# jayin92/Skyfall-GS

Hardware: AMD Instinct MI355X
Metric: train-step Gaussians/s (fwd+bwd raster) @1080p (higher is better)
Workload: dtype f32; 1 GPU; configs[1]: synthetic cfg2 scene (SURVEY 8d), N=2000000 Gaussians/GPU, 1920x1080, z ~ U(250, 350), colors_precomp, kernel_size=0.1, subpixel_offset=zeros[H,W,2], dL/dimage and dL/ddepth ~ N(0,1)/P, seed=rank, one scene per GPU; N=2000000, width=1920, height=1080, N_vis=2000000, D_ref_16x16=5856939, D_binned_8x8=6945415, parallelism=scene-per-gpu x1, prewarm_steps=50, settle_steps=0, order=random

## Files before the change

### skyfall-gs_amd/csrc/raster_bwd.hip

```cpp
#include <cstring>

#include "act_math.h"
#include "sfgs_internal.h"

namespace sfgs {

__global__ void __launch_bounds__(256)
dupgrad_prefill_kernel(int T8, const uint16_t* __restrict__ tile_dead, unsigned long long n_dup, int mode,
                       uint4* __restrict__ live16, uint4* __restrict__ zero_line, unsigned long long* __restrict__ hdr,
                       unsigned long long* __restrict__ feedback, const unsigned long long* __restrict__ dup_pool,
                       unsigned long long dup_capacity, unsigned npools) {
  __shared__ unsigned part[4];
  unsigned dead = 0;
  unsigned long long dead64 = 0ull;
  const uint4* v = reinterpret_cast<const uint4*>(tile_dead);
  const int n8 = T8 / 8;
  for (int i = threadIdx.x; i < n8; i += 256) {
    const uint4 q = v[i];
    dead += (q.x & 0xffffu) + (q.x >> 16) + (q.y & 0xffffu) + (q.y >> 16) + (q.z & 0xffffu) + (q.z >> 16) +
            (q.w & 0xffffu) + (q.w >> 16);
    if (dead > 0x7fffffffu) { dead64 += dead; dead = 0; }
  }
  for (int t = n8 * 8 + threadIdx.x; t < T8; t += 256) dead += tile_dead[t];
  dead64 += dead;
// ... 61 lines not shown
    __syncthreads();
    if (lane == 0) {
#pragma unroll
      for (int i = 0; i < NF; ++i) part[wave][i] = v[i];
    }
    __syncthreads();
    if (threadIdx.x < NF) {
      const float s = ((part[0][threadIdx.x] + part[1][threadIdx.x]) + part[2][threadIdx.x]) + part[3][threadIdx.x];
      reinterpret_cast<float*>(dupgrad + d0 * DG_F4)[threadIdx.x] = s;
    }
  }
}

struct DupAcc {
  float4 q[DG_F4];
  __device__ __forceinline__ void zero() {
#pragma unroll
    for (int i = 0; i < DG_F4; ++i) q[i] = make_float4(0.f, 0.f, 0.f, 0.f);
  }
  __device__ __forceinline__ void add(const float4* __restrict__ r) {
#pragma unroll
    for (int i = 0; i < DG_F4; ++i) {
      const float4 x = r[i];
      q[i].x += x.x; q[i].y += x.y; q[i].z += x.z;
      if (DG_F4 == 3) q[i].w += x.w;
    }
  }
  __device__ __forceinline__ float get(int f) const {
    if constexpr (DG_F4 == 3) { const float4 v = q[f >> 2]; const int c = f & 3; return c == 0 ? v.x : c == 1 ? v.y : c == 2 ? v.z : v.w; }
    else { const float4 v = q[f & 3]; const int c = f >> 2; return c == 0 ? v.x : c == 1 ? v.y : v.z; }
  }
};

template <int K, int DEG, bool RAW, int CMX>
__global__ void __launch_bounds__(PRE_BLOCK)
preprocess_bwd_kernel(KFrame kf, int N, const float* __restrict__ means3D, const float* __restrict__ scales,
                      const float* __restrict__ rots, const void* __restrict__ opac_, const void* __restrict__ filt,
                      int raw_mask, const float* __restrict__ shs, const float* __restrict__ shs_rest,
                      const float* __restrict__ sh_dirs, int dirs_are_centers,
                      const int* __restrict__ radii,
                      const uint2* __restrict__ dup, const float4* __restrict__ dupgrad, const uint8_t* __restrict__ live,
                      size_t zero_f4, const unsigned long long* __restrict__ hdr,
                      float* __restrict__ g_means3D, float* __restrict__ g_means2D, float* __restrict__ g_scales,
                      float* __restrict__ g_rots, void* __restrict__ g_opac_, float* __restrict__ g_colors,
                      float* __restrict__ g_shs, float* __restrict__ g_shs_rest, float* __restrict__ g_sh_dirs) {
  constexpr bool SPLIT = CMX >= 3;
  constexpr int CM = SPLIT ? CMX - 3 : CMX;
  static_assert(!SPLIT || (K > 1 && CM != 1), "split SH storage: more than one coefficient, coefficient-major");
  constexpr int PB_CHUNK = 128;
  static_assert((PB_CHUNK * DG_F4) % 64 == 0, "whole load rounds");
  __shared__ float4 pb_stage[PRE_BLOCK / 64][PB_CHUNK * DG_F4];
  const int g = blockIdx.x * PRE_BLOCK + threadIdx.x;
  const bool valid = g < N;
  const int lane = threadIdx.x & 63;
  constexpr unsigned COOP = 32;
  const bool vis = valid && radii[g] > 0;
  unsigned d0 = 0, cnt = 0;
  if (vis) { const uint2 dr = dup[g]; d0 = dr.x; cnt = dr.y; }
  const bool flags = live != nullptr && hdr[HDR_PREFILLED] != 0ull;
  DupAcc acc;
  acc.zero();
  if (cnt > BWD_BIG) {
    for (unsigned d = d0; d < d0 + cnt; d += BWD_CHUNK) acc.add(dupgrad + (size_t)d * DG_F4);
  }
  {
    const bool small = cnt > 0 && cnt <= COOP;
    const unsigned rb = small ? d0 : 0xffffffffu, re = small ? d0 + cnt : 0u;
    unsigned w0 = rb, w1 = re;
#pragma unroll
    for (int d = 32; d >= 1; d >>= 1) {
      w0 = min(w0, (unsigned)__shfl_xor((int)w0, d));
      w1 = max(w1, (unsigned)__shfl_xor((int)w1, d));
    }
    float4* stage = pb_stage[threadIdx.x >> 6];
    for (unsigned c0 = w0; c0 < w1; c0 += PB_CHUNK) {
      const unsigned c1 = min(c0 + PB_CHUNK, w1);
      if (__ballot(small && rb < c1 && re > c0) == 0ull) continue;
      const unsigned n4 = (c1 - c0) * DG_F4;
      constexpr int NLD = PB_CHUNK * DG_F4 / 64;
      float4 tmp[NLD];
      size_t src[NLD];
#pragma unroll
      for (int k = 0; k < NLD; ++k) src[k] = (size_t)c0 * DG_F4 + min((unsigned)(k * 64 + lane), n4 - 1u);
      if (flags) {
        static_assert(DG_F4 == 3, "piece -> record: u / 3");
        unsigned char lv[NLD];
#pragma unroll
        for (int k = 0; k < NLD; ++k) lv[k] = live[(size_t)c0 + min((unsigned)(k * 64 + lane), n4 - 1u) / 3u];
        unsigned any = 0;
#pragma unroll
        for (int k = 0; k < NLD; ++k) { src[k] = lv[k] ? src[k] : zero_f4; any |= lv[k]; }
        if (__ballot(any != 0u) == 0ull) continue;
      }
#pragma unroll
      for (int k = 0; k < NLD; ++k) tmp[k] = dupgrad[src[k]];
#pragma unroll
      for (int k = 0; k < NLD; ++k) stage[k * 64 + lane] = tmp[k];
      __builtin_amdgcn_wave_barrier();
      __builtin_amdgcn_fence(__ATOMIC_ACQ_REL, "wavefront");
      if (small) {
        const unsigned lo = max(rb, c0), hi = min(re, c1);
        for (unsigned d = lo; d < hi; ++d) acc.add(stage + (size_t)(d - c0) * DG_F4);
      }
      __builtin_amdgcn_wave_barrier();
      __builtin_amdgcn_fence(__ATOMIC_ACQ_REL, "wavefront");
    }
  }
  for (unsigned long long todo = __ballot(cnt > COOP && cnt <= BWD_BIG); todo; todo &= todo - 1) {
    const int src = __builtin_ctzll(todo);
    const unsigned b0 = (unsigned)__shfl((int)d0, src), bn = (unsigned)__shfl((int)cnt, src);
    DupAcc w;
    w.zero();
    if (flags) {
      constexpr int U = 4;
      for (unsigned r = 0; r < bn; r += 64 * U) {
        bool lv[U];
        bool any = false;
#pragma unroll
        for (int j = 0; j < U; ++j) {
          const unsigned i = r + 64u * j + lane;
          lv[j] = live[(size_t)b0 + min(i, bn - 1u)] != 0 && i < bn;
          any |= lv[j];
        }
        if (__ballot(any) == 0ull) continue;
#pragma unroll
        for (int j = 0; j < U; ++j)
          if (lv[j]) w.add(dupgrad + (size_t)(b0 + r + 64u * j + lane) * DG_F4);
      }
    } else {
      for (unsigned i = lane; i < bn; i += 64) w.add(dupgrad + (size_t)(b0 + i) * DG_F4);
    }
#pragma unroll
    for (int i = 0; i < DG_F4; ++i) {
#pragma unroll
      for (int d = 32; d >= 1; d >>= 1) {
        w.q[i].x += __shfl_xor(w.q[i].x, d); w.q[i].y += __shfl_xor(w.q[i].y, d); w.q[i].z += __shfl_xor(w.q[i].z, d);
        if (DG_F4 == 3) w.q[i].w += __shfl_xor(w.q[i].w, d);
      }
    }
    if (lane == src) acc = w;
  }
  if (!valid) return;
  FrameParams f = load_frame(kf);
  f.sh_degree = DEG; f.sh_coeffs = K;
  GaussGrads out;
#pragma unroll
  for (int i = 0; i < 3; ++i) { out.means3D[i] = 0.f; out.means2D[i] = 0.f; out.scales[i] = 0.f; out.rgb[i] = 0.f; }
#pragma unroll
  for (int i = 0; i < 4; ++i) out.rot[i] = 0.f;
  out.opacity = 0.f;
  constexpr int ROW = K > 0 ? 3 * K : 1;
  float gshl[ROW];
#pragma unroll
  for (int i = 0; i < ROW; ++i) gshl[i] = 0.f;
  float gdir[3] = {0.f, 0.f, 0.f};
  if (vis) {
    GradSums A;
    A.x = acc.get(0); A.y = acc.get(1); A.ax = acc.get(2); A.ay = acc.get(3);
    A.xx = acc.get(4); A.xy = acc.get(5); A.yy = acc.get(6); A.u = acc.get(7);
    A.r = acc.get(8); A.g = acc.get(9); A.b = acc.get(10); A.d = acc.get(11);
    float p[3], s[3];
    load3(means3D + 3 * (size_t)g, p);
    load3(scales + 3 * (size_t)g, s);
    const float4 qraw = *reinterpret_cast<const float4*>(rots + 4 * (size_t)g);
    float4 qv = qraw;
    float opacity;
    const float sraw[3] = {s[0], s[1], s[2]};
    unsigned long long o_bits = 0ull, f_bits = 0ull;
    if constexpr (!RAW) {
      opacity = static_cast<const float*>(opac_)[g];
    } else {
#define SFGS_ACT_LOAD(FT, OT) do { o_bits = raw_bits<OT>(opac_, g); f_bits = raw_bits<FT>(filt, g); } while (0)
      SFGS_ACT_DISPATCH(raw_mask, SFGS_ACT_LOAD);
#undef SFGS_ACT_LOAD
#define SFGS_ACT_FWD(FT, OT) act_outputs(act_terms<FT, OT>(sraw, from_bits<OT>(o_bits), from_bits<FT>(f_bits)), s, &opacity)
      SFGS_ACT_DISPATCH(raw_mask, SFGS_ACT_FWD);
#undef SFGS_ACT_FWD
      qv = act_rotation(qraw);
    }
    const float q[4] = {qv.x, qv.y, qv.z, qv.w};
    if constexpr (K > 0) {
      float shl[ROW];
      if constexpr (SPLIT) load_sh_rows<K>(shs, shs_rest, (size_t)g, shl);
      else load_row<ROW>(shs + (size_t)ROW * g, shl);
      if constexpr (CM != 0) {
        float din[3];
        load3(sh_dirs + 3 * (size_t)g, din);
        preprocess_backward_sums(f, p, s, q, opacity, shl, A, out, gshl, CM == 1, dirs_are_centers ? nullptr : din, gdir,
                                 dirs_are_centers ? din : nullptr);
      } else {
        preprocess_backward_sums(f, p, s, q, opacity, shl, A, out, gshl);
      }
    } else {
      preprocess_backward_sums(f, p, s, q, opacity, nullptr, A, out, gshl);
    }
    if constexpr (RAW) {
      const float gs[3] = {out.scales[0], out.scales[1], out.scales[2]};
#define SFGS_ACT_BWD(FT, OT)                                                                                         \
  do {                                                                                                              \
    OT gro;                                                                                                         \
    act_backward(act_terms<FT, OT>(sraw, from_bits<OT>(o_bits), from_bits<FT>(f_bits)), gs, out.opacity, out.scales, \
                 &gro);                                                                                             \
    static_cast<OT*>(g_opac_)[g] = gro;                                                                             \
  } while (0)
      SFGS_ACT_DISPATCH(raw_mask, SFGS_ACT_BWD);
#undef SFGS_ACT_BWD
      const float4 gq = act_rotation_backward(qraw, make_float4(out.rot[0], out.rot[1], out.rot[2], out.rot[3]));
// ... 136 lines not shown
```

### skyfall-gs_amd/csrc/raster_preprocess.hip

```cpp
#include <algorithm>

#include "act_math.h"
#include "sfgs_internal.h"

namespace sfgs {


__global__ void __launch_bounds__(256) subpix_bound_kernel(const float* __restrict__ subpix, int64_t n,
                                                           unsigned long long* __restrict__ hdr) {
  __shared__ float s_m[4];
  float m = 0.f;
  const int64_t n4 = (reinterpret_cast<uintptr_t>(subpix) & 15) ? 0 : (n >> 2);
  const float4* __restrict__ v4 = reinterpret_cast<const float4*>(subpix);
  for (int64_t i = (int64_t)blockIdx.x * blockDim.x + threadIdx.x; i < n4; i += (int64_t)gridDim.x * blockDim.x) {
    const float4 v = v4[i];
    m = fmaxf(fmaxf(m, fmaxf(fabsf(v.x), fabsf(v.y))), fmaxf(fabsf(v.z), fabsf(v.w)));
  }
  for (int64_t i = (n4 << 2) + (int64_t)blockIdx.x * blockDim.x + threadIdx.x; i < n; i += (int64_t)gridDim.x * blockDim.x)
    m = fmaxf(m, fabsf(subpix[i]));
#pragma unroll
  for (int d = 32; d >= 1; d >>= 1) m = fmaxf(m, __shfl_xor(m, d));
  if (lane_id() == 0) s_m[threadIdx.x >> 6] = m;
  __syncthreads();
  if (threadIdx.x == 0) {
// ... 45 lines not shown
  bool hit = false;
  int cb = 0;
  if (i < ncb) {
    const int cx = a.cx0 + i % nx, cy = a.cy0 + i / nx;
    const int tx = cx * COARSE + (t & (COARSE - 1)), ty = cy * COARSE + (t / COARSE);
    cb = cy * CX + cx;
    if (tx >= a.br.x0 && tx < a.br.x1 && ty >= a.br.y0 && ty < a.br.y1) hit = bin_test(a.r, a.thr, tx, ty, W, H, bound);
  }
  *cb_index = cb;
  return __ballot(hit);
}

__device__ __forceinline__ unsigned wave_sum_u32(unsigned v) {
#pragma unroll
  for (int d = 32; d >= 1; d >>= 1) v += (unsigned)__shfl_xor((int)v, d);
  return v;
}

template <int K, int DEG, bool RAW, int CM>
__global__ void __launch_bounds__(PRE_BLOCK)
preprocess_kernel(KFrame kf, int N, const float* __restrict__ means3D, const float* __restrict__ scales,
                  const float* __restrict__ rots, const void* __restrict__ opac_, const void* __restrict__ filt,
                  int raw_mask,
                  const float* __restrict__ colors, const float* __restrict__ shs, const float* __restrict__ shs_rest,
                  const float* __restrict__ sh_dirs, int dirs_are_centers, int* __restrict__ radii,
                  float4* __restrict__ rec_out, uint2* __restrict__ dup_out, uint32_t* __restrict__ coarse_count,
                  uint4* __restrict__ slabs, unsigned coarse_capacity, unsigned long long dup_capacity,
                  uint32_t* __restrict__ block_nvis, unsigned long long* __restrict__ block_dref,
                  uint4* __restrict__ big_list, unsigned long long* __restrict__ hdr,
                  unsigned long long* __restrict__ dup_pool, uint4* __restrict__ pairs,
                  uint32_t* __restrict__ block_items) {
  __shared__ unsigned s_red[PRE_BLOCK / 64 + 1];
  __shared__ unsigned long long s_base;
  const FrameParams f = load_frame(kf);
  const float bound = __uint_as_float((unsigned)hdr[HDR_SUBPIX_BOUND]);
  const int g = blockIdx.x * PRE_BLOCK + threadIdx.x;
  const int CX = (((f.W + TILE_BIN - 1) / TILE_BIN) + COARSE - 1) / COARSE;
  unsigned n_dup = 0, vis = 0, dref = 0, depth_bits = 0;
  unsigned long long mask_lo = 0ull, mask_hi = 0ull;
  unsigned walk_tiles = 0;
  bool big = false;
  bool huge = false;
  const int lane = threadIdx.x & 63;
  SplatRec r;
  BinRange br;
  float thr = 0.f;
  int cx0 = 0, cx1 = 0, cy0 = 0, cy1 = 0;
  br.x0 = br.x1 = br.y0 = br.y1 = 0;
  if (g < N) {
    float p[3], s[3];
    load3(means3D + 3 * (size_t)g, p);
    load3(scales + 3 * (size_t)g, s);
    float4 qv = *reinterpret_cast<const float4*>(rots + 4 * (size_t)g);
    float opacity_in = 0.f;
    if constexpr (!RAW) opacity_in = static_cast<const float*>(opac_)[g];
    float rgb_in[3] = {0.f, 0.f, 0.f};
    if constexpr (K == 0) load3(colors + 3 * (size_t)g, rgb_in);
    unsigned long long o_bits = 0ull, f_bits = 0ull;
    if constexpr (RAW) {
#define SFGS_ACT_LOAD(FT, OT) do { o_bits = raw_bits<OT>(opac_, g); f_bits = raw_bits<FT>(filt, g); } while (0)
      SFGS_ACT_DISPATCH(raw_mask, SFGS_ACT_LOAD);
#undef SFGS_ACT_LOAD
    }
    asm volatile("" :: "v"(p[2]), "v"(s[0]), "v"(qv.x), "v"(opacity_in), "v"(rgb_in[0]), "v"((unsigned)o_bits),
                 "v"((unsigned)f_bits));
    if constexpr (RAW) {
// ... 111 lines not shown
      __builtin_amdgcn_wave_barrier();
    }
  }
  const unsigned long long big_lanes = __ballot(big);
  for (unsigned long long bl = big_lanes; bl; bl &= bl - 1) {
    const int L = __builtin_ctzll(bl);
    const WalkArgs a = broadcast_walk(r, br, thr, cx0, cx1, cy0, cy1, L);
    const int ncb = (a.cx1 - a.cx0) * (a.cy1 - a.cy0);
    unsigned total = 0;
    for (int it = 0; it * 4 < ncb; ++it) {
      int cb;
      total += (unsigned)__popcll(walk_ballot4(a, it, lane, f.W, f.H, bound, &cb, CX));
    }
    if (lane == L) n_dup = total;
  }
  const unsigned long long huge_lanes = __ballot(huge);
  if (huge_lanes) {
    unsigned long long slot0 = 0ull;
    if (lane == 0) slot0 = atomicAdd(&hdr[HDR_BIG_COUNT], (unsigned long long)__popcll(huge_lanes));
    const unsigned s_lo = (unsigned)__builtin_amdgcn_readfirstlane((int)(unsigned)slot0);
    if (huge) {
      const unsigned rk = __builtin_amdgcn_mbcnt_hi((unsigned)(huge_lanes >> 32), __builtin_amdgcn_mbcnt_lo((unsigned)huge_lanes, 0u));
      big_list[s_lo + rk] = make_uint4((unsigned)g, (unsigned)br.x0 | ((unsigned)br.x1 << 16),
                                       (unsigned)br.y0 | ((unsigned)br.y1 << 16), 0u);
    }
  }
  unsigned n_items = 0;
  if (pairs && n_dup && !big && !huge) {
#pragma unroll
    for (int k = 0; k < BIG_WALK; ++k)
      n_items += ((k < 4 ? mask_lo >> (16 * k) : mask_hi >> (16 * (k - 4))) & 0xffffull) != 0ull;
  }
  static_assert(PAIRS_PER_BLOCK == PRE_BLOCK * BIG_WALK, "a thread emits at most BIG_WALK items itself");
  unsigned total;
  const unsigned ex_packed = block_excl_scan_u32<PRE_BLOCK>(n_dup | (n_items << 20), &total, s_red);
  const unsigned ex = ex_packed & 0xfffffu, ex_items = ex_packed >> 20, total_items = total >> 20;
  total &= 0xfffffu;
  __shared__ int s_fits;
  if (threadIdx.x == 0) {
    bool ok = true;
    s_base = total ? dup_alloc(dup_pool, dup_pools_used(gridDim.x), blockIdx.x, total, dup_capacity, &ok) : 0ull;
    s_fits = ok;
  }
  __syncthreads();
  const unsigned long long base = s_base;
  const bool fits = s_fits != 0;
  if (!fits && threadIdx.x == 0) hdr[HDR_OVERFLOW] = 1ull;
  if (g < N && !huge) dup_out[g] = make_uint2((unsigned)(base + ex), n_dup);
  {
    const bool emit = fits && n_dup && !big;
    const int nb = emit ? (cx1 - cx0) * (cy1 - cy0) : 0;
    unsigned dup = (unsigned)(base + ex);
    int cx = cx0, cy = cy0;
    if (pairs) {
      unsigned pos = blockIdx.x * (unsigned)PAIRS_PER_BLOCK + ex_items;
#pragma unroll
      for (int k = 0; k < BIG_WALK; ++k) {
        if (k < nb) {
          const unsigned m = (unsigned)((k < 4 ? mask_lo >> (16 * k) : mask_hi >> (16 * (k - 4))) & 0xffffull);
          if (m) {
            pairs[pos++] = make_uint4((unsigned)g, depth_bits, dup, m | ((unsigned)(cy * CX + cx) << 16));
            dup += (unsigned)__popc(m);
          }
          if (++cx == cx1) { cx = cx0; ++cy; }
        }
      }
      if (threadIdx.x == 0) block_items[blockIdx.x] = fits ? total_items : 0u;
    } else {
    const unsigned long long le = (2ull << lane) - 1ull;
    for (int k = 0; __ballot(k < nb) != 0ull; ++k) {
      unsigned m = 0;
      if (k < nb) m = (unsigned)((k < 4 ? mask_lo >> (16 * k) : mask_hi >> (16 * (k - 4))) & 0xffffull);
      const int cb = cy * CX + cx;
      const unsigned key = m ? (unsigned)cb : 0x80000000u | (unsigned)lane;
      const unsigned prev = (unsigned)__shfl_up((int)key, 1);
      const unsigned long long heads = __ballot(lane == 0 || key != prev);
      const int h = 63 - __clzll(heads & le);
      const unsigned long long above = heads & ~le;
      const int next = above ? __ffsll((long long)above) - 1 : 64;
      const unsigned pc = m ? (unsigned)__popc(m) : 0u;
// ... 14 lines not shown
        dup += (unsigned)__popc(m);
      }
      if (k < nb && ++cx == cx1) { cx = cx0; ++cy; }
    }
    }
  }
  for (unsigned long long bl = fits ? big_lanes : 0ull; bl; bl &= bl - 1) {
    const int L = __builtin_ctzll(bl);
    const WalkArgs a = broadcast_walk(r, br, thr, cx0, cx1, cy0, cy1, L);
    const unsigned g_L = (unsigned)__shfl((int)g, L), depth_L = __shfl(depth_bits, L);
    unsigned dup = __shfl((unsigned)(base + ex), L);
    const int ncb = (a.cx1 - a.cx0) * (a.cy1 - a.cy0);
    const int q = lane >> 4, turn = lane & 15;
    const unsigned long long below_q = (1ull << (16 * q)) - 1ull;
    unsigned m_mine = 0u, dp_mine = 0u;
    int cb_mine = 0;
    for (int it = 0; it * 4 < ncb; ++it) {
      int cb;
      const unsigned long long bal = walk_ballot4(a, it, lane, f.W, f.H, bound, &cb, CX);
      if (turn == it) {
        m_mine = (unsigned)(bal >> (16 * q)) & 0xffffu;
        cb_mine = cb;
        dp_mine = dup + (unsigned)__popcll(bal & below_q);
      }
      dup += (unsigned)__popcll(bal);
    }
    if (m_mine) {
      const unsigned rank = (unsigned)atomicAdd(reinterpret_cast<unsigned long long*>(&coarse_count[(size_t)cb_mine * CC_STRIDE]),
                                                1ull | ((unsigned long long)(unsigned)__popc(m_mine) << 32));
      if (rank < coarse_capacity) slabs[(size_t)cb_mine * coarse_capacity + rank] = make_uint4(g_L, depth_L, dp_mine, m_mine);
      else hdr[HDR_OVERFLOW] = 1ull;
    }
  }
  block_excl_scan_u32<PRE_BLOCK>(vis, &total, s_red);
  if (threadIdx.x == 0) block_nvis[blockIdx.x] = total;
  block_excl_scan_u32<PRE_BLOCK>(dref, &total, s_red);
  if (threadIdx.x == 0) block_dref[blockIdx.x] = total;
}

__global__ void __launch_bounds__(256)
big_walk_kernel(KFrame kf, const uint4* __restrict__ big_list, const float4* __restrict__ rec,
                uint2* __restrict__ dup_out, uint32_t* __restrict__ coarse_count, uint4* __restrict__ slabs,
                unsigned coarse_capacity, unsigned long long dup_capacity, uint2* __restrict__ big_chunks,
                unsigned big_chunk_cap, unsigned long long* __restrict__ hdr, unsigned long long* __restrict__ dup_pool,
                unsigned npools) {
  __shared__ uint16_t bw_masks[4][BIG_WALK_CACHE];
  uint16_t* my_masks = bw_masks[threadIdx.x >> 6];
  const unsigned n_big = (unsigned)hdr[HDR_BIG_COUNT];
  const int lane = threadIdx.x & 63;
  const unsigned nwaves = gridDim.x * (blockDim.x >> 6);
  const int W = kf.W, H = kf.H;
  const int CX = (((W + TILE_BIN - 1) / TILE_BIN) + COARSE - 1) / COARSE;
  const float bound = __uint_as_float((unsigned)hdr[HDR_SUBPIX_BOUND]);
  for (unsigned i = blockIdx.x * (blockDim.x >> 6) + (threadIdx.x >> 6); i < n_big; i += nwaves) {
    const uint4 it = big_list[i];
    const unsigned g = it.x;
    const float4 r0 = rec[REC_F4 * (size_t)g], r1 = rec[REC_F4 * (size_t)g + 1], r2 = rec[REC_F4 * (size_t)g + 2];
    WalkArgs a;
    a.r.mx = r0.x; a.r.my = r0.y; a.r.qa = r0.z; a.r.qb = r0.w; a.r.qc = r1.x; a.r.op = r1.y; a.r.depth = r2.y;
    a.r.r = a.r.g = a.r.b = 0.f; a.r.ex = r2.z; a.r.ey = r2.w;
    a.br.x0 = (int)(it.y & 0xffffu); a.br.x1 = (int)(it.y >> 16);
    a.br.y0 = (int)(it.z & 0xffffu); a.br.y1 = (int)(it.z >> 16);
    a.thr = alpha_threshold_log2(a.r.op);
    a.cx0 = a.br.x0 / COARSE; a.cx1 = (a.br.x1 - 1) / COARSE + 1;
    a.cy0 = a.br.y0 / COARSE; a.cy1 = (a.br.y1 - 1) / COARSE + 1;
    const unsigned depth_bits = __float_as_uint(a.r.depth);
    const int nx = a.cx1 - a.cx0, ncb = nx * (a.cy1 - a.cy0);
    unsigned total = 0;
    for (int i0 = 0; i0 < ncb; i0 += 64) {
      const int j = i0 + lane;
// ... 104 lines not shown
```

### skyfall-gs_amd/csrc/raster_binning.hip

```cpp
#include <algorithm>

#include "sfgs_internal.h"

namespace sfgs {

constexpr int SCATTER_NT = 1024, SCATTER_BINS = 4096, SCATTER_IDX = 15360, SCATTER_MLP = 4;
static_assert(SCATTER_BLOCKS * PAIRS_PER_BLOCK <= 65536, "16-bit pair indices");
static_assert(SCATTER_BLOCKS <= 64, "one wave scans the block counts");

__device__ __forceinline__ unsigned scatter_prefix(const uint32_t* __restrict__ block_items, int b0, int nblk,
                                                   unsigned* s_prefix) {
  const int tid = threadIdx.x;
  if (tid < 64) {
    const unsigned c = tid < nblk ? block_items[b0 + tid] : 0u;
    const unsigned incl = wave_incl_scan_u32(c);
    if (tid < SCATTER_BLOCKS) s_prefix[tid + 1] = incl;
    if (tid == 0) s_prefix[0] = 0u;
  }
  __syncthreads();
  return s_prefix[nblk];
}
__device__ __forceinline__ const uint4* scatter_pair(const uint4* __restrict__ pairs, const unsigned* s_prefix, int b0,
                                                     int nblk, unsigned i) {
  int lo = 0, hi = nblk;
#pragma unroll
  for (int it = 0; it < 6; ++it) {
    const int mid = (lo + hi) >> 1;
    if (hi - lo > 1) { if (s_prefix[mid] <= i) lo = mid; else hi = mid; }
  }
  return pairs + (size_t)(b0 + lo) * PAIRS_PER_BLOCK + (i - s_prefix[lo]);
}

__global__ void __launch_bounds__(SCATTER_NT)
bin_count_kernel(int NB, int NCB, const uint4* __restrict__ pairs, const uint32_t* __restrict__ block_items,
                 uint32_t* __restrict__ sc_cnt, uint32_t* __restrict__ sc_hits) {
  __shared__ unsigned s_prefix[SCATTER_BLOCKS + 1];
  __shared__ unsigned s_items[SCATTER_BINS], s_hits[SCATTER_BINS];
  const int tid = threadIdx.x;
  const int b0 = blockIdx.x * SCATTER_BLOCKS, nblk = min(SCATTER_BLOCKS, NB - b0);
  const unsigned total = scatter_prefix(block_items, b0, nblk, s_prefix);
  for (int r0 = 0; r0 < NCB; r0 += SCATTER_BINS) {
    const int nbins = min(SCATTER_BINS, NCB - r0);
    for (int i = tid; i < nbins; i += SCATTER_NT) { s_items[i] = 0u; s_hits[i] = 0u; }
    __syncthreads();
    for (unsigned i0 = tid; i0 < total; i0 += SCATTER_MLP * SCATTER_NT) {
      unsigned w[SCATTER_MLP];
#pragma unroll
      for (int u = 0; u < SCATTER_MLP; ++u)
        w[u] = i0 + u * SCATTER_NT < total ? scatter_pair(pairs, s_prefix, b0, nblk, i0 + u * SCATTER_NT)->w : 0u;
#pragma unroll
      for (int u = 0; u < SCATTER_MLP; ++u) {
        const int cb = (int)(w[u] >> 16) - r0;
        if ((w[u] & 0xffffu) && cb >= 0 && cb < nbins) {
          atomicAdd(&s_items[cb], 1u);
          atomicAdd(&s_hits[cb], (unsigned)__popc(w[u] & 0xffffu));
        }
      }
    }
    __syncthreads();
    for (int i = tid; i < nbins; i += SCATTER_NT) {
      sc_cnt[(size_t)blockIdx.x * NCB + r0 + i] = s_items[i];
      sc_hits[(size_t)blockIdx.x * NCB + r0 + i] = s_hits[i];
    }
    __syncthreads();
  }
}

constexpr int RANK_COLS = 16, RANK_GROUPS = 64;
__device__ __forceinline__ int rank_row(int k, int NWG) {
  const int q = NWG >> 3, r = NWG & 7;
  int x = 0, first = 0;
#pragma unroll
  for (int t = 1; t < 8; ++t) {
    const int st = min(t, r) * (q + 1) + max(t - r, 0) * q;
    if (k >= st) { x = t; first = st; }
  }
  return (k - first) * 8 + x;
}
__global__ void __launch_bounds__(RANK_COLS * RANK_GROUPS)
bin_rank_kernel(int NWG, int NCB, const uint32_t* __restrict__ sc_cnt, const uint32_t* __restrict__ sc_hits,
                uint32_t* __restrict__ sc_base, uint32_t* __restrict__ coarse_count, unsigned long long* __restrict__ hdr) {
  __shared__ unsigned s_c[RANK_GROUPS][RANK_COLS], s_h[RANK_GROUPS][RANK_COLS];
  __shared__ unsigned s_tot[RANK_COLS], s_first[RANK_COLS];
  const int c = threadIdx.x % RANK_COLS, g = threadIdx.x / RANK_COLS;
  const int bin = min(blockIdx.x * RANK_COLS + c, NCB - 1);
  const bool live = blockIdx.x * RANK_COLS + c < NCB;
  const int R = (NWG + RANK_GROUPS - 1) / RANK_GROUPS;
  const int w0 = min(g * R, NWG), w1 = min(w0 + R, NWG);
  unsigned long long* counter = reinterpret_cast<unsigned long long*>(&coarse_count[(size_t)bin * CC_STRIDE]);
  const unsigned long long old = *counter;
  unsigned sc = 0u, sh = 0u;
  for (int w = w0; w < w1; w += 4) {
    unsigned tc[4], th[4];
#pragma unroll
    for (int u = 0; u < 4; ++u) {
      const size_t at = (size_t)rank_row(min(w + u, w1 - 1), NWG) * NCB + bin;
      tc[u] = sc_cnt[at]; th[u] = sc_hits[at];
    }
#pragma unroll
    for (int u = 0; u < 4; ++u)
      if (w + u < w1) { sc += tc[u]; sh += th[u]; }
  }
  s_c[g][c] = sc; s_h[g][c] = sh;
  __syncthreads();
  if (g == 0) {
    unsigned tot = 0u;
    for (int q = 0; q < RANK_GROUPS; ++q) tot += s_c[q][c];
    s_tot[c] = live ? tot : 0u;
  }
  __syncthreads();
  if (threadIdx.x == 0) {
    unsigned sum = 0u;
#pragma unroll
    for (int k = 0; k < RANK_COLS; ++k) { s_first[k] = sum; sum += s_tot[k]; }
    const unsigned at = (unsigned)atomicAdd(&hdr[HDR_CSR_CURSOR], (unsigned long long)sum);
#pragma unroll
    for (int k = 0; k < RANK_COLS; ++k) s_first[k] += at;
  }
  __syncthreads();
  unsigned run = s_first[c];
  for (int q = 0; q < g; ++q) run += s_c[q][c];
  for (int w = w0; w < w1; w += 4) {
    unsigned tc[4];
#pragma unroll
    for (int u = 0; u < 4; ++u) tc[u] = sc_cnt[(size_t)rank_row(min(w + u, w1 - 1), NWG) * NCB + bin];
#pragma unroll
    for (int u = 0; u < 4; ++u)
      if (w + u < w1) {
        if (live) sc_base[(size_t)rank_row(w + u, NWG) * NCB + bin] = run;
        run += tc[u];
      }
  }
  if (g == RANK_GROUPS - 1 && live) {
    unsigned hits = (unsigned)(old >> 32);
    for (int q = 0; q < RANK_GROUPS; ++q) hits += s_h[q][c];
    *counter = (unsigned long long)((unsigned)old + s_tot[c]) | ((unsigned long long)hits << 32);
    coarse_count[(size_t)bin * CC_STRIDE + 6] = s_first[c];
    coarse_count[(size_t)bin * CC_STRIDE + 7] = s_tot[c];
  }
}

__device__ void plan_scan_role(int role, int NCB, int NB, uint32_t* __restrict__ coarse_count,
                               const uint32_t* __restrict__ block_nvis, const unsigned long long* __restrict__ block_dref,
                               unsigned long long* __restrict__ hdr, const unsigned long long* __restrict__ feedback,
                               const unsigned long long* __restrict__ dup_pool, unsigned long long* __restrict__ host_out,
                               unsigned coarse_capacity);

__global__ void __launch_bounds__(SCATTER_NT)
bin_scatter_kernel(int NB, int NCB, const uint4* __restrict__ pairs, const uint32_t* __restrict__ block_items,
                   const uint32_t* __restrict__ sc_cnt, const uint32_t* __restrict__ sc_base,
                   uint4* __restrict__ csr, unsigned csr_capacity, unsigned coarse_capacity,
                   unsigned long long* __restrict__ hdr, int plan_roles, uint32_t* __restrict__ coarse_count, const uint32_t* __restrict__ block_nvis,
                   const unsigned long long* __restrict__ block_dref, const unsigned long long* __restrict__ feedback,
                   const unsigned long long* __restrict__ dup_pool, unsigned long long* __restrict__ host_out) {
  const int n_scatter = (int)gridDim.x - plan_roles;
  if ((int)blockIdx.x >= n_scatter) {
    plan_scan_role((int)blockIdx.x - n_scatter, NCB, NB, coarse_count, block_nvis, block_dref, hdr, feedback, dup_pool,
                   host_out, coarse_capacity);
    return;
  }
  const int wg = (int)blockIdx.x;
  __shared__ unsigned s_prefix[SCATTER_BLOCKS + 1];
  __shared__ unsigned s_red[SCATTER_NT / 64 + 1];
  __shared__ unsigned s_delta[SCATTER_BINS];
  __shared__ unsigned s_cur[SCATTER_BINS];
  __shared__ unsigned short s_idx[SCATTER_IDX];
  const int tid = threadIdx.x;
  const int b0 = wg * SCATTER_BLOCKS, nblk = min(SCATTER_BLOCKS, NB - b0);
  const unsigned total = scatter_prefix(block_items, b0, nblk, s_prefix);
  if (total == 0u) return;
  for (int r0 = 0; r0 < NCB; r0 += SCATTER_BINS) {
    const int nbins = min(SCATTER_BINS, NCB - r0);
    static_assert(SCATTER_BINS <= 4 * SCATTER_NT, "four bins per thread");
    unsigned c[4], base[4];
#pragma unroll
    for (int u = 0; u < 4; ++u) {
      const int i = tid + u * SCATTER_NT;
      c[u] = i < nbins ? sc_cnt[(size_t)wg * NCB + r0 + i] : 0u;
      base[u] = i < nbins ? sc_base[(size_t)wg * NCB + r0 + i] : 0u;
    }
    unsigned round_total;
    unsigned p = block_excl_scan_u32<SCATTER_NT>(c[0] + c[1] + c[2] + c[3], &round_total, s_red);
#pragma unroll
    for (int u = 0; u < 4; ++u) {
      const int i = tid + u * SCATTER_NT;
      if (i < nbins) { s_delta[i] = base[u] - p; s_cur[i] = p; }
      p += c[u];
    }
    __syncthreads();
    for (unsigned i0 = tid; i0 < total; i0 += SCATTER_MLP * SCATTER_NT) {
      uint4 it[SCATTER_MLP];
#pragma unroll
      for (int u = 0; u < SCATTER_MLP; ++u)
        it[u] = i0 + u * SCATTER_NT < total ? *scatter_pair(pairs, s_prefix, b0, nblk, i0 + u * SCATTER_NT)
                                            : make_uint4(0u, 0u, 0u, 0u);
#pragma unroll
      for (int u = 0; u < SCATTER_MLP; ++u) {
        const unsigned m = it[u].w & 0xffffu;
        const int cb = (int)(it[u].w >> 16) - r0;
        if (m && cb >= 0 && cb < nbins) {
          const unsigned pos = atomicAdd(&s_cur[cb], 1u);
          if (pos < (unsigned)SCATTER_IDX) {
            s_idx[pos] = (unsigned short)(i0 + u * SCATTER_NT);
          } else {
            const unsigned at = s_delta[cb] + pos;
            if (at < csr_capacity) csr[at] = make_uint4(it[u].x, it[u].y, it[u].z, m);
            else hdr[HDR_OVERFLOW] = 1ull;
          }
        }
      }
    }
    __syncthreads();
    const unsigned nsorted = min(round_total, (unsigned)SCATTER_IDX);
    for (unsigned q0 = tid; q0 < nsorted; q0 += SCATTER_MLP * SCATTER_NT) {
      uint4 it[SCATTER_MLP];
#pragma unroll
      for (int u = 0; u < SCATTER_MLP; ++u)
        it[u] = q0 + u * SCATTER_NT < nsorted ? *scatter_pair(pairs, s_prefix, b0, nblk, s_idx[q0 + u * SCATTER_NT])
                                              : make_uint4(0u, 0u, 0u, 0u);
#pragma unroll
      for (int u = 0; u < SCATTER_MLP; ++u) {
        if (q0 + u * SCATTER_NT < nsorted) {
          const int cb = (int)(it[u].w >> 16) - r0;
          const unsigned at = s_delta[cb] + (q0 + u * SCATTER_NT);
          if (at < csr_capacity) csr[at] = make_uint4(it[u].x, it[u].y, it[u].z, it[u].w & 0xffffu);
          else hdr[HDR_OVERFLOW] = 1ull;
        }
      }
    }
    __syncthreads();
  }
}

__device__ void bin_base_scan(int NCB, uint32_t* __restrict__ coarse_count, unsigned long long* __restrict__ hdr) {
  __shared__ unsigned long long bb_wave[17];
  const int nt = blockDim.x, lane = threadIdx.x & 63, wave = threadIdx.x >> 6, nw = nt >> 6;
  unsigned long long carry = 0;
  for (int c0 = 0; c0 < NCB; c0 += nt) {
    const int cb = c0 + threadIdx.x;
    const unsigned need = cb < NCB ? bin_slots_needed(coarse_count[(size_t)cb * CC_STRIDE + 1]) : 0u;
    unsigned long long incl = need;
#pragma unroll
    for (int o = 1; o < 64; o <<= 1) { const unsigned long long t = __shfl_up(incl, o); if (lane >= o) incl += t; }
    __syncthreads();
    if (lane == 63) bb_wave[wave] = incl;
    __syncthreads();
    unsigned long long before = carry, all = 0;
    for (int w = 0; w < nw; ++w) { const unsigned long long t = bb_wave[w]; if (w < wave) before += t; all += t; }
    if (cb < NCB) coarse_count[(size_t)cb * CC_STRIDE + 2] = (unsigned)min(before + incl - need, 0xffffffffull);
    carry += all;
  }
  if (threadIdx.x == 0) hdr[HDR_ITEM_ALLOC] = carry;
// ... 236 lines not shown
```

Baseline: 2.256 billion Gaussians/s.

## Stage dup gradients via direct global-to-LDS loads and hoist per-Gaussian loads

In the backward preprocess kernel, the cooperative dup-gradient staging now uses global_load_lds to copy straight from global memory into LDS instead of going through registers. The chunk size grows from 128 to 256, with explicit vmcnt/lgkmcnt waits in place of implicit dependencies. Per-Gaussian parameter loads (means, scales, rotation, opacity, radii, dup) are hoisted to the top of the kernel so their latency overlaps the gradient reduction. In the preprocess kernel, the two trailing block scans for visible and dref counts become wave-level reductions written through shared memory, removing extra block synchronisation; the cost is a doubled LDS footprint and more live registers, which may lower occupancy.

After: 2.270 billion Gaussians/s, median of 6. Within noise of the previous version (+0.6%).

```diff
diff --git a/skyfall-gs_amd/csrc/raster_bwd.hip b/skyfall-gs_amd/csrc/raster_bwd.hip
--- a/skyfall-gs_amd/csrc/raster_bwd.hip
+++ b/skyfall-gs_amd/csrc/raster_bwd.hip
@@ -117,6 +117,17 @@
   }
 };
 
+__device__ __forceinline__ void load_to_lds16(const float4* src, float4* dst) {
+  __builtin_amdgcn_global_load_lds((const __attribute__((address_space(1))) void*)src,
+                                   (__attribute__((address_space(3))) void*)dst, 16, 0, 0);
+}
+template <int N_>
+__device__ __forceinline__ void wait_vm() {
+  static_assert(N_ >= 0 && N_ < 64, "vmcnt has six bits");
+  __builtin_amdgcn_s_waitcnt(0x0f70 | (N_ & 15) | ((N_ >> 4) << 14));
+}
+__device__ __forceinline__ void wait_lds_reads() { __builtin_amdgcn_s_waitcnt(0xc07f); }
+
 template <int K, int DEG, bool RAW, int CMX>
 __global__ void __launch_bounds__(PRE_BLOCK)
 preprocess_bwd_kernel(KFrame kf, int N, const float* __restrict__ means3D, const float* __restrict__ scales,
@@ -132,16 +143,32 @@
   constexpr bool SPLIT = CMX >= 3;
   constexpr int CM = SPLIT ? CMX - 3 : CMX;
   static_assert(!SPLIT || (K > 1 && CM != 1), "split SH storage: more than one coefficient, coefficient-major");
-  constexpr int PB_CHUNK = 128;
+  constexpr int PB_CHUNK = 256;
   static_assert((PB_CHUNK * DG_F4) % 64 == 0, "whole load rounds");
   __shared__ float4 pb_stage[PRE_BLOCK / 64][PB_CHUNK * DG_F4];
   const int g = blockIdx.x * PRE_BLOCK + threadIdx.x;
   const bool valid = g < N;
   const int lane = threadIdx.x & 63;
+  const int gc = min(g, N - 1);
+  const int rad_in = radii[gc];
+  const uint2 dr_in = dup[gc];
+  float p[3], s[3];
+  load3(means3D + 3 * (size_t)gc, p);
+  load3(scales + 3 * (size_t)gc, s);
+  const float4 qraw = *reinterpret_cast<const float4*>(rots + 4 * (size_t)gc);
+  float opacity = 0.f;
+  unsigned long long o_bits = 0ull, f_bits = 0ull;
+  if constexpr (!RAW) {
+    opacity = static_cast<const float*>(opac_)[gc];
+  } else {
+#define SFGS_ACT_LOAD(FT, OT) do { o_bits = raw_bits<OT>(opac_, gc); f_bits = raw_bits<FT>(filt, gc); } while (0)
+    SFGS_ACT_DISPATCH(raw_mask, SFGS_ACT_LOAD);
+#undef SFGS_ACT_LOAD
+  }
   constexpr unsigned COOP = 32;
-  const bool vis = valid && radii[g] > 0;
+  const bool vis = valid && rad_in > 0;
   unsigned d0 = 0, cnt = 0;
-  if (vis) { const uint2 dr = dup[g]; d0 = dr.x; cnt = dr.y; }
+  if (vis) { d0 = dr_in.x; cnt = dr_in.y; }
   const bool flags = live != nullptr && hdr[HDR_PREFILLED] != 0ull;
   DupAcc acc;
   acc.zero();
@@ -157,36 +184,41 @@
       w0 = min(w0, (unsigned)__shfl_xor((int)w0, d));
       w1 = max(w1, (unsigned)__shfl_xor((int)w1, d));
     }
-    float4* stage = pb_stage[threadIdx.x >> 6];
-    for (unsigned c0 = w0; c0 < w1; c0 += PB_CHUNK) {
-      const unsigned c1 = min(c0 + PB_CHUNK, w1);
+    const unsigned sw0 = (unsigned)__builtin_amdgcn_readfirstlane((int)w0), sw1 = (unsigned)__builtin_amdgcn_readfirstlane((int)w1);
+    float4* stage = pb_stage[__builtin_amdgcn_readfirstlane((int)(threadIdx.x >> 6))];
+    for (unsigned c0 = sw0; c0 < sw1; c0 += PB_CHUNK) {
+      const unsigned c1 = min(c0 + PB_CHUNK, sw1);
       if (__ballot(small && rb < c1 && re > c0) == 0ull) continue;
       const unsigned n4 = (c1 - c0) * DG_F4;
       constexpr int NLD = PB_CHUNK * DG_F4 / 64;
-      float4 tmp[NLD];
-      size_t src[NLD];
-#pragma unroll
-      for (int k = 0; k < NLD; ++k) src[k] = (size_t)c0 * DG_F4 + min((unsigned)(k * 64 + lane), n4 - 1u);
+      const float4* wsrc = dupgrad + (size_t)c0 * DG_F4;
       if (flags) {
         static_assert(DG_F4 == 3, "piece -> record: u / 3");
+        static_assert(NLD <= 32, "one flag bit per load");
+        const uint8_t* wlive = live + (size_t)c0;
         unsigned char lv[NLD];
 #pragma unroll
-        for (int k = 0; k < NLD; ++k) lv[k] = live[(size_t)c0 + min((unsigned)(k * 64 + lane), n4 - 1u) / 3u];
-        unsigned any = 0;
-#pragma unroll
-        for (int k = 0; k < NLD; ++k) { src[k] = lv[k] ? src[k] : zero_f4; any |= lv[k]; }
-        if (__ballot(any != 0u) == 0ull) continue;
-      }
-#pragma unroll
-      for (int k = 0; k < NLD; ++k) tmp[k] = dupgrad[src[k]];
-#pragma unroll
-      for (int k = 0; k < NLD; ++k) stage[k * 64 + lane] = tmp[k];
+        for (int k = 0; k < NLD; ++k) lv[k] = wlive[min((unsigned)(k * 64 + lane), n4 - 1u) / 3u];
+        unsigned lmask = 0;
+#pragma unroll
+        for (int k = 0; k < NLD; ++k) lmask |= (lv[k] ? 1u : 0u) << k;
+        if (__ballot(lmask != 0u) == 0ull) continue;
+        const float4* zsrc = dupgrad + zero_f4;
+#pragma unroll
+        for (int k = 0; k < NLD; ++k)
+          load_to_lds16((lmask >> k) & 1u ? wsrc + min((unsigned)(k * 64 + lane), n4 - 1u) : zsrc, stage + k * 64);
+      } else {
+#pragma unroll
+        for (int k = 0; k < NLD; ++k) load_to_lds16(wsrc + min((unsigned)(k * 64 + lane), n4 - 1u), stage + k * 64);
+      }
+      wait_vm<0>();
       __builtin_amdgcn_wave_barrier();
       __builtin_amdgcn_fence(__ATOMIC_ACQ_REL, "wavefront");
       if (small) {
         const unsigned lo = max(rb, c0), hi = min(re, c1);
         for (unsigned d = lo; d < hi; ++d) acc.add(stage + (size_t)(d - c0) * DG_F4);
       }
+      wait_lds_reads();
       __builtin_amdgcn_wave_barrier();
       __builtin_amdgcn_fence(__ATOMIC_ACQ_REL, "wavefront");
     }
@@ -244,20 +276,9 @@
     A.x = acc.get(0); A.y = acc.get(1); A.ax = acc.get(2); A.ay = acc.get(3);
     A.xx = acc.get(4); A.xy = acc.get(5); A.yy = acc.get(6); A.u = acc.get(7);
     A.r = acc.get(8); A.g = acc.get(9); A.b = acc.get(10); A.d = acc.get(11);
-    float p[3], s[3];
-    load3(means3D + 3 * (size_t)g, p);
-    load3(scales + 3 * (size_t)g, s);
-    const float4 qraw = *reinterpret_cast<const float4*>(rots + 4 * (size_t)g);
     float4 qv = qraw;
-    float opacity;
     const float sraw[3] = {s[0], s[1], s[2]};
-    unsigned long long o_bits = 0ull, f_bits = 0ull;
-    if constexpr (!RAW) {
-      opacity = static_cast<const float*>(opac_)[g];
-    } else {
-#define SFGS_ACT_LOAD(FT, OT) do { o_bits = raw_bits<OT>(opac_, g); f_bits = raw_bits<FT>(filt, g); } while (0)
-      SFGS_ACT_DISPATCH(raw_mask, SFGS_ACT_LOAD);
-#undef SFGS_ACT_LOAD
+    if constexpr (RAW) {
 #define SFGS_ACT_FWD(FT, OT) act_outputs(act_terms<FT, OT>(sraw, from_bits<OT>(o_bits), from_bits<FT>(f_bits)), s, &opacity)
       SFGS_ACT_DISPATCH(raw_mask, SFGS_ACT_FWD);
 #undef SFGS_ACT_FWD
diff --git a/skyfall-gs_amd/csrc/raster_preprocess.hip b/skyfall-gs_amd/csrc/raster_preprocess.hip
--- a/skyfall-gs_amd/csrc/raster_preprocess.hip
+++ b/skyfall-gs_amd/csrc/raster_preprocess.hip
@@ -101,6 +101,7 @@
                   uint32_t* __restrict__ block_items) {
   __shared__ unsigned s_red[PRE_BLOCK / 64 + 1];
   __shared__ unsigned long long s_base;
+  __shared__ unsigned s_stat[2][PRE_BLOCK / 64];
   const FrameParams f = load_frame(kf);
   const float bound = __uint_as_float((unsigned)hdr[HDR_SUBPIX_BOUND]);
   const int g = blockIdx.x * PRE_BLOCK + threadIdx.x;
@@ -278,6 +279,10 @@
       n_items += ((k < 4 ? mask_lo >> (16 * k) : mask_hi >> (16 * (k - 4))) & 0xffffull) != 0ull;
   }
   static_assert(PAIRS_PER_BLOCK == PRE_BLOCK * BIG_WALK, "a thread emits at most BIG_WALK items itself");
+  {
+    const unsigned nv = (unsigned)__popcll(__ballot(vis != 0u)), dr = wave_sum_u32(dref);
+    if ((threadIdx.x & 63) == 0) { s_stat[0][threadIdx.x >> 6] = nv; s_stat[1][threadIdx.x >> 6] = dr; }
+  }
   unsigned total;
   const unsigned ex_packed = block_excl_scan_u32<PRE_BLOCK>(n_dup | (n_items << 20), &total, s_red);
   const unsigned ex = ex_packed & 0xfffffu, ex_items = ex_packed >> 20, total_items = total >> 20;
@@ -292,6 +297,13 @@
   const unsigned long long base = s_base;
   const bool fits = s_fits != 0;
   if (!fits && threadIdx.x == 0) hdr[HDR_OVERFLOW] = 1ull;
+  if (threadIdx.x == 0) {
+    unsigned nv = 0, dr = 0;
+#pragma unroll
+    for (int w = 0; w < PRE_BLOCK / 64; ++w) { nv += s_stat[0][w]; dr += s_stat[1][w]; }
+    block_nvis[blockIdx.x] = nv;
+    block_dref[blockIdx.x] = dr;
+  }
   if (g < N && !huge) dup_out[g] = make_uint2((unsigned)(base + ex), n_dup);
   {
     const bool emit = fits && n_dup && !big;
@@ -372,10 +384,6 @@
       else hdr[HDR_OVERFLOW] = 1ull;
     }
   }
-  block_excl_scan_u32<PRE_BLOCK>(vis, &total, s_red);
-  if (threadIdx.x == 0) block_nvis[blockIdx.x] = total;
-  block_excl_scan_u32<PRE_BLOCK>(dref, &total, s_red);
-  if (threadIdx.x == 0) block_dref[blockIdx.x] = total;
 }
 
 __global__ void __launch_bounds__(256)
```

## Walk preprocess blocks directly in binning kernels instead of prefix-search indexing

Applied to the files above, without the earlier changes.

Replaces the per-item binary search over a shared prefix of per-block pair counts with a fixed mapping: each half-wave of 32 threads strides through one preprocess block's pairs. The sorted-index pass now stores padded block-local indices, so the second pass reads pairs directly without a search. The rank kernel also keeps the first-pass counts in registers when each group handles at most four rows, avoiding a reread. The cost is load imbalance when block item counts differ, since threads assigned to sparse blocks sit idle.

Result: slower. 2.225 billion Gaussians/s before, 2.198 billion Gaussians/s after (-1.2%).

```diff
diff --git a/skyfall-gs_amd/csrc/raster_binning.hip b/skyfall-gs_amd/csrc/raster_binning.hip
--- a/skyfall-gs_amd/csrc/raster_binning.hip
+++ b/skyfall-gs_amd/csrc/raster_binning.hip
@@ -6,50 +6,44 @@
 
 constexpr int SCATTER_NT = 1024, SCATTER_BINS = 4096, SCATTER_IDX = 15360, SCATTER_MLP = 4;
 static_assert(SCATTER_BLOCKS * PAIRS_PER_BLOCK <= 65536, "16-bit pair indices");
-static_assert(SCATTER_BLOCKS <= 64, "one wave scans the block counts");
-
-__device__ __forceinline__ unsigned scatter_prefix(const uint32_t* __restrict__ block_items, int b0, int nblk,
-                                                   unsigned* s_prefix) {
-  const int tid = threadIdx.x;
-  if (tid < 64) {
-    const unsigned c = tid < nblk ? block_items[b0 + tid] : 0u;
-    const unsigned incl = wave_incl_scan_u32(c);
-    if (tid < SCATTER_BLOCKS) s_prefix[tid + 1] = incl;
-    if (tid == 0) s_prefix[0] = 0u;
-  }
-  __syncthreads();
-  return s_prefix[nblk];
-}
-__device__ __forceinline__ const uint4* scatter_pair(const uint4* __restrict__ pairs, const unsigned* s_prefix, int b0,
-                                                     int nblk, unsigned i) {
-  int lo = 0, hi = nblk;
-#pragma unroll
-  for (int it = 0; it < 6; ++it) {
-    const int mid = (lo + hi) >> 1;
-    if (hi - lo > 1) { if (s_prefix[mid] <= i) lo = mid; else hi = mid; }
-  }
-  return pairs + (size_t)(b0 + lo) * PAIRS_PER_BLOCK + (i - s_prefix[lo]);
+
+constexpr int SCATTER_SUB = SCATTER_NT / SCATTER_BLOCKS;
+static_assert(SCATTER_SUB * SCATTER_BLOCKS == SCATTER_NT && SCATTER_SUB == 32, "half a wave per preprocess block");
+struct BlockWalk {
+  const uint4* src;
+  unsigned cnt;
+  unsigned first;
+  unsigned sub;
+};
+__device__ __forceinline__ BlockWalk block_walk(const uint4* __restrict__ pairs, const uint32_t* __restrict__ block_items,
+                                                int b0, int nblk) {
+  const int blk = (int)threadIdx.x / SCATTER_SUB;
+  BlockWalk w;
+  w.src = pairs + (size_t)(b0 + min(blk, nblk - 1)) * PAIRS_PER_BLOCK;
+  w.cnt = blk < nblk ? min(block_items[b0 + blk], (unsigned)PAIRS_PER_BLOCK) : 0u;
+  w.first = (unsigned)blk * PAIRS_PER_BLOCK;
+  w.sub = threadIdx.x % SCATTER_SUB;
+  return w;
 }
 
 __global__ void __launch_bounds__(SCATTER_NT)
 bin_count_kernel(int NB, int NCB, const uint4* __restrict__ pairs, const uint32_t* __restrict__ block_items,
                  uint32_t* __restrict__ sc_cnt, uint32_t* __restrict__ sc_hits) {
-  __shared__ unsigned s_prefix[SCATTER_BLOCKS + 1];
   __shared__ unsigned s_items[SCATTER_BINS], s_hits[SCATTER_BINS];
   const int tid = threadIdx.x;
   const int b0 = blockIdx.x * SCATTER_BLOCKS, nblk = min(SCATTER_BLOCKS, NB - b0);
-  const unsigned total = scatter_prefix(block_items, b0, nblk, s_prefix);
+  const BlockWalk bw = block_walk(pairs, block_items, b0, nblk);
   for (int r0 = 0; r0 < NCB; r0 += SCATTER_BINS) {
     const int nbins = min(SCATTER_BINS, NCB - r0);
     for (int i = tid; i < nbins; i += SCATTER_NT) { s_items[i] = 0u; s_hits[i] = 0u; }
     __syncthreads();
-    for (unsigned i0 = tid; i0 < total; i0 += SCATTER_MLP * SCATTER_NT) {
+    for (unsigned k0 = bw.sub; k0 < bw.cnt; k0 += SCATTER_MLP * SCATTER_SUB) {
       unsigned w[SCATTER_MLP];
 #pragma unroll
-      for (int u = 0; u < SCATTER_MLP; ++u)
-        w[u] = i0 + u * SCATTER_NT < total ? scatter_pair(pairs, s_prefix, b0, nblk, i0 + u * SCATTER_NT)->w : 0u;
+      for (int u = 0; u < SCATTER_MLP; ++u) w[u] = bw.src[min(k0 + u * SCATTER_SUB, bw.cnt - 1u)].w;
 #pragma unroll
       for (int u = 0; u < SCATTER_MLP; ++u) {
+        if (k0 + u * SCATTER_SUB >= bw.cnt) w[u] = 0u;
         const int cb = (int)(w[u] >> 16) - r0;
         if ((w[u] & 0xffffu) && cb >= 0 && cb < nbins) {
           atomicAdd(&s_items[cb], 1u);
@@ -90,6 +84,7 @@
   unsigned long long* counter = reinterpret_cast<unsigned long long*>(&coarse_count[(size_t)bin * CC_STRIDE]);
   const unsigned long long old = *counter;
   unsigned sc = 0u, sh = 0u;
+  unsigned keep[4] = {0u, 0u, 0u, 0u};
   for (int w = w0; w < w1; w += 4) {
     unsigned tc[4], th[4];
 #pragma unroll
@@ -98,8 +93,10 @@
       tc[u] = sc_cnt[at]; th[u] = sc_hits[at];
     }
 #pragma unroll
-    for (int u = 0; u < 4; ++u)
+    for (int u = 0; u < 4; ++u) {
+      keep[u] = tc[u];
       if (w + u < w1) { sc += tc[u]; sh += th[u]; }
+    }
   }
   s_c[g][c] = sc; s_h[g][c] = sh;
   __syncthreads();
@@ -122,8 +119,13 @@
   for (int q = 0; q < g; ++q) run += s_c[q][c];
   for (int w = w0; w < w1; w += 4) {
     unsigned tc[4];
-#pragma unroll
-    for (int u = 0; u < 4; ++u) tc[u] = sc_cnt[(size_t)rank_row(min(w + u, w1 - 1), NWG) * NCB + bin];
+    if (R <= 4) {
+#pragma unroll
+      for (int u = 0; u < 4; ++u) tc[u] = keep[u];
+    } else {
+#pragma unroll
+      for (int u = 0; u < 4; ++u) tc[u] = sc_cnt[(size_t)rank_row(min(w + u, w1 - 1), NWG) * NCB + bin];
+    }
 #pragma unroll
     for (int u = 0; u < 4; ++u)
       if (w + u < w1) {
@@ -160,15 +162,15 @@
     return;
   }
   const int wg = (int)blockIdx.x;
-  __shared__ unsigned s_prefix[SCATTER_BLOCKS + 1];
   __shared__ unsigned s_red[SCATTER_NT / 64 + 1];
   __shared__ unsigned s_delta[SCATTER_BINS];
   __shared__ unsigned s_cur[SCATTER_BINS];
   __shared__ unsigned short s_idx[SCATTER_IDX];
   const int tid = threadIdx.x;
   const int b0 = wg * SCATTER_BLOCKS, nblk = min(SCATTER_BLOCKS, NB - b0);
-  const unsigned total = scatter_prefix(block_items, b0, nblk, s_prefix);
-  if (total == 0u) return;
+  const BlockWalk bw = block_walk(pairs, block_items, b0, nblk);
+  const uint4* __restrict__ wg_pairs = pairs + (size_t)b0 * PAIRS_PER_BLOCK;
+  if (!__syncthreads_or(bw.cnt != 0u)) return;
   for (int r0 = 0; r0 < NCB; r0 += SCATTER_BINS) {
     const int nbins = min(SCATTER_BINS, NCB - r0);
     static_assert(SCATTER_BINS <= 4 * SCATTER_NT, "four bins per thread");
@@ -188,20 +190,19 @@
       p += c[u];
     }
     __syncthreads();
-    for (unsigned i0 = tid; i0 < total; i0 += SCATTER_MLP * SCATTER_NT) {
+    for (unsigned k0 = bw.sub; k0 < bw.cnt; k0 += SCATTER_MLP * SCATTER_SUB) {
       uint4 it[SCATTER_MLP];
 #pragma unroll
-      for (int u = 0; u < SCATTER_MLP; ++u)
-        it[u] = i0 + u * SCATTER_NT < total ? *scatter_pair(pairs, s_prefix, b0, nblk, i0 + u * SCATTER_NT)
-                                            : make_uint4(0u, 0u, 0u, 0u);
+      for (int u = 0; u < SCATTER_MLP; ++u) it[u] = bw.src[min(k0 + u * SCATTER_SUB, bw.cnt - 1u)];
 #pragma unroll
       for (int u = 0; u < SCATTER_MLP; ++u) {
-        const unsigned m = it[u].w & 0xffffu;
+        const unsigned k = k0 + u * SCATTER_SUB;
+        const unsigned m = k < bw.cnt ? it[u].w & 0xffffu : 0u;
         const int cb = (int)(it[u].w >> 16) - r0;
         if (m && cb >= 0 && cb < nbins) {
           const unsigned pos = atomicAdd(&s_cur[cb], 1u);
           if (pos < (unsigned)SCATTER_IDX) {
-            s_idx[pos] = (unsigned short)(i0 + u * SCATTER_NT);
+            s_idx[pos] = (unsigned short)(bw.first + k);
           } else {
             const unsigned at = s_delta[cb] + pos;
             if (at < csr_capacity) csr[at] = make_uint4(it[u].x, it[u].y, it[u].z, m);
@@ -215,9 +216,7 @@
     for (unsigned q0 = tid; q0 < nsorted; q0 += SCATTER_MLP * SCATTER_NT) {
       uint4 it[SCATTER_MLP];
 #pragma unroll
-      for (int u = 0; u < SCATTER_MLP; ++u)
-        it[u] = q0 + u * SCATTER_NT < nsorted ? *scatter_pair(pairs, s_prefix, b0, nblk, s_idx[q0 + u * SCATTER_NT])
-                                              : make_uint4(0u, 0u, 0u, 0u);
+      for (int u = 0; u < SCATTER_MLP; ++u) it[u] = wg_pairs[s_idx[min(q0 + u * SCATTER_NT, nsorted - 1u)]];
 #pragma unroll
       for (int u = 0; u < SCATTER_MLP; ++u) {
         if (q0 + u * SCATTER_NT < nsorted) {
```
